# qcraftai/gedepth

Measured on AMD Instinct MI355X. Metric: training img/s (whole node), KITTI-shaped 352x1120 synthetic batches, higher is better.
Workload: dtype bf16; 1 GPU; depthformer_swint_v: DepthFormer-SwinT + GEDepth-Vanilla, 352x1120, 8 img/GPU, full train step; global_batch=8, parallelism=dp1, allreduce_dtype=fp32, layout=nhwc, window_attention=bf16 mfma, params=53516992, hip_graph=off

## Files before the change

gedepth_amd/csrc/conv3x3.hip:

```cpp
#include "common.h"
#include <stdlib.h>

typedef __bf16 cv_bf16x8 __attribute__((ext_vector_type(8)));
typedef float cv_f32x16 __attribute__((ext_vector_type(16)));

#define CV_TH 8
#define CV_TW 32
#define CV_KC 32
#define CV_PITCH 40
#define CV_HALO ((CV_TH + 2) * (CV_TW + 2))
#define CV_NT 64
#define CV_IN_PIECES (CV_HALO * 4)
#define CV_W_PIECES (9 * CV_NT * 4)

__global__ void __launch_bounds__(256, 2) conv3x3_nhwc_k(const bf16_t* __restrict__ x, const bf16_t* __restrict__ w, const float* __restrict__ bias,
                                                         bf16_t* __restrict__ y, int H, int W, int Cin, int Cout, int n_ntiles, float slope,
                                                         int act) {
  __shared__ __attribute__((aligned(16))) bf16_t smem[CV_HALO * CV_PITCH + 9 * CV_NT * CV_PITCH];
  bf16_t* in_tile = smem;
  bf16_t* w_tile = smem + CV_HALO * CV_PITCH;
  const int tid = threadIdx.x, lane = tid & 63, wv = tid >> 6;
  const int tx0 = blockIdx.x * CV_TW, ty0 = blockIdx.y * CV_TH;
  const int n = blockIdx.z / n_ntiles, n0 = (blockIdx.z - n * n_ntiles) * CV_NT;
  const bf16_t* xn = x + (long)n * H * W * Cin;

  int in_src[6], in_dst[6], w_src[9], w_dst[9];
#pragma unroll
  for (int i = 0; i < 6; ++i) {
    const int p = tid + i * 256;
    in_src[i] = -1; in_dst[i] = 0;
    if (p < CV_IN_PIECES) {
      const int pix = p >> 2, part = p & 3;
      const int iy = pix / (CV_TW + 2), ix = pix - iy * (CV_TW + 2);
      const int gy = ty0 + iy - 1, gx = tx0 + ix - 1;
      in_dst[i] = pix * CV_PITCH + part * 8;
      in_src[i] = (gy >= 0 && gy < H && gx >= 0 && gx < W) ? (gy * W + gx) * Cin + part * 8 : -2;
    }
  }
#pragma unroll
  for (int i = 0; i < 9; ++i) {
    const int p = tid + i * 256;
    const int row = p >> 2, part = p & 3;
    const int tap = row / CV_NT, co = row - tap * CV_NT;
    w_dst[i] = row * CV_PITCH + part * 8;
    w_src[i] = (n0 + co < Cout) ? ((n0 + co) * 9 + tap) * Cin + part * 8 : -2;
  }
  uint4 pin[6], pw[9];
  const uint4 zero4 = make_uint4(0, 0, 0, 0);
#define CV_PREFETCH(C0)                                                                          \
  _Pragma("unroll") for (int i = 0; i < 6; ++i) { pin[i] = zero4; if (in_src[i] >= 0) pin[i] = *(const uint4*)(xn + in_src[i] + (C0)); } \
  _Pragma("unroll") for (int i = 0; i < 9; ++i) { pw[i] = zero4; if (w_src[i] >= 0) pw[i] = *(const uint4*)(w + w_src[i] + (C0)); }
#define CV_PARK()                                                                                \
  _Pragma("unroll") for (int i = 0; i < 6; ++i) if (in_src[i] != -1) *(uint4*)(in_tile + in_dst[i]) = pin[i];             \
  _Pragma("unroll") for (int i = 0; i < 9; ++i) *(uint4*)(w_tile + w_dst[i]) = pw[i];

  cv_f32x16 acc[2][2];
#pragma unroll
  for (int a = 0; a < 2; ++a)
#pragma unroll
    for (int b = 0; b < 2; ++b) acc[a][b] = 0.f;
  const int m = lane & 31, kg = lane >> 5;
  const int a_base0 = ((2 * wv) * (CV_TW + 2) + m) * CV_PITCH + kg * 8;
  const int b_base = m * CV_PITCH + kg * 8;

  CV_PREFETCH(0)
  CV_PARK()
  __syncthreads();
  for (int c0 = 0; c0 < Cin; c0 += CV_KC) {
    const bool more = c0 + CV_KC < Cin;
    if (more) { CV_PREFETCH(c0 + CV_KC) }
    {
      cv_bf16x8 A[2][2], B[2][2];
      auto frags = [&](int set, int it) {
        const int tap = it >> 1, ks = it & 1, r = tap / 3, s = tap - 3 * r;
        const int ao = a_base0 + (r * (CV_TW + 2) + s) * CV_PITCH + ks * 16;
        A[set][0] = *(const cv_bf16x8*)(in_tile + ao);
        A[set][1] = *(const cv_bf16x8*)(in_tile + ao + (CV_TW + 2) * CV_PITCH);
        const int bo = b_base + tap * CV_NT * CV_PITCH + ks * 16;
        B[set][0] = *(const cv_bf16x8*)(w_tile + bo);
        B[set][1] = *(const cv_bf16x8*)(w_tile + bo + 32 * CV_PITCH);
      };
      frags(0, 0);
#pragma unroll
      for (int it = 0; it < 18; ++it) {
        if (it < 17) frags((it + 1) & 1, it + 1);
        __builtin_amdgcn_sched_barrier(0);
        const int c = it & 1;
        acc[0][0] = __builtin_amdgcn_mfma_f32_32x32x16_bf16(A[c][0], B[c][0], acc[0][0], 0, 0, 0);
        acc[0][1] = __builtin_amdgcn_mfma_f32_32x32x16_bf16(A[c][0], B[c][1], acc[0][1], 0, 0, 0);
        acc[1][0] = __builtin_amdgcn_mfma_f32_32x32x16_bf16(A[c][1], B[c][0], acc[1][0], 0, 0, 0);
        acc[1][1] = __builtin_amdgcn_mfma_f32_32x32x16_bf16(A[c][1], B[c][1], acc[1][1], 0, 0, 0);
        __builtin_amdgcn_sched_barrier(0);
      }
    }
    __syncthreads();
    if (more) { CV_PARK() }
    __syncthreads();
  }
#undef CV_PREFETCH
#undef CV_PARK

  bf16_t* ot = smem + wv * (64 * 72);
#pragma unroll
  for (int mb = 0; mb < 2; ++mb)
#pragma unroll
    for (int nb = 0; nb < 2; ++nb) {
      const int co = nb * 32 + m;
      const float bv = (bias && n0 + co < Cout) ? bias[n0 + co] : 0.f;
#pragma unroll
      for (int r = 0; r < 16; ++r) {
        float v = acc[mb][nb][r] + bv;
        if (act) v = v > 0.f ? v : v * slope;
        const int px = (r & 3) + 8 * (r >> 2) + 4 * kg;
        ot[(mb * 32 + px) * 72 + co] = __builtin_bit_cast(bf16_t, (__bf16)v);
      }
    }
  __builtin_amdgcn_wave_barrier();
#pragma unroll
  for (int it = 0; it < 8; ++it) {
    const int p = it * 8 + (lane >> 3), piece = lane & 7;
    const int gy = ty0 + 2 * wv + (p >> 5), gx = tx0 + (p & 31);
    if (gy < H && gx < W && n0 + piece * 8 < Cout)
      *(uint4*)(y + (((long)n * H + gy) * W + gx) * Cout + n0 + piece * 8) = *(const uint4*)(ot + p * 72 + piece * 8);
  }
}

#define CD_TH 16
#define CD_TW 32
#define CD_HP ((CD_TH + 2) * (CD_TW + 2))
#define CD_HCH 39
#define CD_WCH 36
#define CD_HB (CD_HCH * 1024)
#define CD_BUF (80 * 1024)
#define CD_NCH (CD_HCH + CD_WCH)
#define CD_SLOTS 10
#define CD_LDS(T, p) ((__attribute__((address_space(3))) T*)(p))
#define CD_GLB(p) ((const __attribute__((address_space(1))) void*)(p))

__device__ __attribute__((aligned(16))) uint32_t cd_zero16[4] = {0, 0, 0, 0};

__global__ void __launch_bounds__(512, 1) conv3x3_nhwc_dma_k(const bf16_t* __restrict__ x, const bf16_t* __restrict__ w, const float* __restrict__ bias,
                                                             bf16_t* __restrict__ y, int H, int W, int Cin, int Cout, int n_ntiles, float slope,
                                                             int act) {
  __shared__ __attribute__((aligned(1024))) unsigned char smem[2 * CD_BUF];
  const int tid = threadIdx.x, lane = tid & 63;
  const int wv = __builtin_amdgcn_readfirstlane(tid >> 6);
  const int tx0 = blockIdx.x * CD_TW, ty0 = blockIdx.y * CD_TH;
  const int n = blockIdx.z / n_ntiles, n0 = (blockIdx.z - n * n_ntiles) * CV_NT;
  const unsigned char* xn = (const unsigned char*)(x + (long)n * H * W * Cin);
  const unsigned char* wb = (const unsigned char*)w;

  unsigned goff[CD_SLOTS];
#pragma unroll
  for (int i = 0; i < CD_SLOTS; ++i) {
    const int ch = wv + 8 * i;
    unsigned off = ~0u;
    if (ch < CD_HCH) {
      const int q = ch * 64 + lane, hp = q >> 2, piece = (q & 3) ^ ((hp >> 2) & 3);
      if (hp < CD_HP) {
        const int iy = hp / (CD_TW + 2), ix = hp - iy * (CD_TW + 2);
        const int gy = ty0 + iy - 1, gx = tx0 + ix - 1;
        if (gy >= 0 && gy < H && gx >= 0 && gx < W) off = (unsigned)(((gy * W + gx) * Cin + piece * 8) * 2);
      }
    } else if (ch < CD_NCH) {
      const int q = (ch - CD_HCH) * 64 + lane, row = q >> 2, piece = (q & 3) ^ ((row >> 2) & 3);
      const int tap = row >> 6, co = row & 63;
      if (n0 + co < Cout) off = (unsigned)((((n0 + co) * 9 + tap) * Cin + piece * 8) * 2);
    }
    goff[i] = off;
  }
  auto dma = [&](int i, int c0, int buf) {
    const int ch = wv + 8 * i;
    const unsigned char* base = ch < CD_HCH ? xn : wb;
    const unsigned char* p = goff[i] == ~0u ? (const unsigned char*)cd_zero16 : base + (size_t)(goff[i] + (unsigned)(c0 * 2));
    const unsigned ldst = (unsigned)(uintptr_t)CD_LDS(unsigned char, smem + buf * CD_BUF + ch * 1024);
    asm volatile("s_mov_b32 m0, %0\n\ts_nop 0\n\tglobal_load_lds_dwordx4 %1, off" :: "s"(ldst), "v"(p) : "memory", "m0");
  };

  cv_f32x16 acc[2][2];
#pragma unroll
  for (int a = 0; a < 2; ++a)
#pragma unroll
    for (int b = 0; b < 2; ++b) acc[a][b] = 0.f;
  const int m = lane & 31, kg = lane >> 5;
  int abase[9][2];
#pragma unroll
  for (int tap = 0; tap < 9; ++tap)
#pragma unroll
    for (int mb = 0; mb < 2; ++mb) {
      const int hp = (2 * wv + mb + tap / 3) * (CD_TW + 2) + m + tap % 3;
      abase[tap][mb] = hp * 64 + ((kg ^ ((hp >> 2) & 3)) << 4);
    }
  const int bbase = CD_HB + m * 64 + ((kg ^ ((m >> 2) & 3)) << 4);

#pragma unroll
  for (int i = 0; i < CD_SLOTS; ++i) dma(i, 0, 0);
  asm volatile("s_waitcnt vmcnt(0)" ::: "memory");
  int buf = 0;
  for (int c0 = 0; c0 < Cin; c0 += CV_KC) {
    asm volatile("" ::: "memory");
    __builtin_amdgcn_s_barrier();
    asm volatile("" ::: "memory");
    const int cn = c0 + CV_KC < Cin ? c0 + CV_KC : c0;
    const unsigned char* base = smem + buf * CD_BUF;
    cv_bf16x8 A[2][2], B[2][2];
    A[0][0] = *(const cv_bf16x8*)(base + abase[0][0]); A[0][1] = *(const cv_bf16x8*)(base + abase[0][1]);
    B[0][0] = *(const cv_bf16x8*)(base + bbase); B[0][1] = *(const cv_bf16x8*)(base + bbase + 2048);
#pragma unroll
    for (int g = 0; g < 18; ++g) {
      const int cs = g & 1, ns = cs ^ 1;
      if (g < 17) {
        const int tap = (g + 1) >> 1, kx = ((g + 1) & 1) << 5;
        A[ns][0] = *(const cv_bf16x8*)(base + (abase[tap][0] ^ kx)); A[ns][1] = *(const cv_bf16x8*)(base + (abase[tap][1] ^ kx));
        B[ns][0] = *(const cv_bf16x8*)(base + (bbase ^ kx) + tap * 4096); B[ns][1] = *(const cv_bf16x8*)(base + (bbase ^ kx) + tap * 4096 + 2048);
      }
      __builtin_amdgcn_sched_barrier(0);
      if (!(g & 1)) dma(g >> 1, cn, buf ^ 1);
      acc[0][0] = __builtin_amdgcn_mfma_f32_32x32x16_bf16(A[cs][0], B[cs][0], acc[0][0], 0, 0, 0);
      acc[0][1] = __builtin_amdgcn_mfma_f32_32x32x16_bf16(A[cs][0], B[cs][1], acc[0][1], 0, 0, 0);
      acc[1][0] = __builtin_amdgcn_mfma_f32_32x32x16_bf16(A[cs][1], B[cs][0], acc[1][0], 0, 0, 0);
      acc[1][1] = __builtin_amdgcn_mfma_f32_32x32x16_bf16(A[cs][1], B[cs][1], acc[1][1], 0, 0, 0);
    }
    dma(9, cn, buf ^ 1);
    asm volatile("s_waitcnt vmcnt(0)" ::: "memory");
    buf ^= 1;
  }
  __builtin_amdgcn_s_barrier();
  asm volatile("" ::: "memory");

  bf16_t* ot = (bf16_t*)smem + wv * (64 * 72);
#pragma unroll
  for (int mb = 0; mb < 2; ++mb)
#pragma unroll
    for (int nb = 0; nb < 2; ++nb) {
      const int co = nb * 32 + m;
      const float bv = (bias && n0 + co < Cout) ? bias[n0 + co] : 0.f;
#pragma unroll
      for (int r = 0; r < 16; ++r) {
        float v = acc[mb][nb][r] + bv;
        if (act) v = v > 0.f ? v : v * slope;
        const int px = (r & 3) + 8 * (r >> 2) + 4 * kg;
        ot[(mb * 32 + px) * 72 + co] = __builtin_bit_cast(bf16_t, (__bf16)v);
      }
    }
  __builtin_amdgcn_wave_barrier();
#pragma unroll
  for (int it = 0; it < 8; ++it) {
    const int p = it * 8 + (lane >> 3), piece = lane & 7;
    const int gy = ty0 + 2 * wv + (p >> 5), gx = tx0 + (p & 31);
    if (gy < H && gx < W && n0 + piece * 8 < Cout)
      *(uint4*)(y + (((long)n * H + gy) * W + gx) * Cout + n0 + piece * 8) = *(const uint4*)(ot + p * 72 + piece * 8);
  }
}

extern "C" int ge_conv3x3_nhwc_fwd(const void* x, const void* w, const float* bias, void* y, int N, int H, int W, int Cin, int Cout, int act,
                                   float slope, int dtype, void* stream) {
  if (!x || !w || !y || N < 0 || H <= 0 || W <= 0 || Cin <= 0 || Cout <= 0) return GE_ERR_BAD_ARG;
  if (dtype != GE_BF16 || Cin % CV_KC || Cout % 8 || (((uintptr_t)x | (uintptr_t)w | (uintptr_t)y) & 15)) return GE_ERR_UNSUPPORTED;
  if ((long)H * W * Cin >= (1L << 31) || (long)Cout * 9 * Cin >= (1L << 31)) return GE_ERR_UNSUPPORTED;
  if (N == 0) return GE_OK;
  const int ntn = (Cout + CV_NT - 1) / CV_NT;
  const char* ev = getenv("GE_CONV3X3");
  const int variant = ev ? atoi(ev) : 0;
  const int hpad16 = (H + CD_TH - 1) / CD_TH * CD_TH, hpad8 = (H + CV_TH - 1) / CV_TH * CV_TH;
  const bool dma = variant == 2 || (variant == 0 && Cin >= 512 && hpad16 * 8 <= hpad8 * 9);
  if (dma) {
    const dim3 grid((W + CD_TW - 1) / CD_TW, (H + CD_TH - 1) / CD_TH, N * ntn);
    if (grid.y > 65535 || grid.z > 65535) return GE_ERR_UNSUPPORTED;
    conv3x3_nhwc_dma_k<<<grid, 512, 0, ge_stream(stream)>>>((const bf16_t*)x, (const bf16_t*)w, bias, (bf16_t*)y, H, W, Cin, Cout, ntn, slope, act);
    GE_LAUNCH_CHECK();
    return GE_OK;
  }
  const dim3 grid((W + CV_TW - 1) / CV_TW, (H + CV_TH - 1) / CV_TH, N * ntn);
  if (grid.y > 65535 || grid.z > 65535) return GE_ERR_UNSUPPORTED;
  conv3x3_nhwc_k<<<grid, 256, 0, ge_stream(stream)>>>((const bf16_t*)x, (const bf16_t*)w, bias, (bf16_t*)y, H, W, Cin, Cout, ntn, slope, act);
  GE_LAUNCH_CHECK();
  return GE_OK;
}
```

gedepth_amd/csrc/conv3x3_wgrad.hip:

```cpp
#include "common.h"

typedef __bf16 wg_bf16x8 __attribute__((ext_vector_type(8)));
typedef __bf16 wg_bf16x4 __attribute__((ext_vector_type(4)));
typedef float wg_f32x16 __attribute__((ext_vector_type(16)));
#define WG_LDS(T, p) ((__attribute__((address_space(3))) T*)(p))

#define WG_TH 8
#define WG_TW 32
#define WG_HALO ((WG_TH + 2) * (WG_TW + 2))
#define WG_PIX (WG_TH * WG_TW)
#define WG_DY_PIECES (WG_PIX * 8)
#define WG_X_PIECES (WG_HALO * 4)

template <int TAP0, int NTAP>
__device__ __forceinline__ void wg_tile_mfma(const bf16_t* dyh, const bf16_t* xt, wg_f32x16* acc) {
  wg_bf16x8 A[2], B[2][NTAP];
#define WG_RD(P) __builtin_shufflevector(__builtin_amdgcn_ds_read_tr16_b64_v4bf16(WG_LDS(wg_bf16x4, (P))), \
                                         __builtin_amdgcn_ds_read_tr16_b64_v4bf16(WG_LDS(wg_bf16x4, (P) + 4 * 32)), 0, 1, 2, 3, 4, 5, 6, 7)
#define WG_FRAGS(SET, KS)                                                                                   \
  {                                                                                                         \
    constexpr int row_ = (KS) >> 1, xh_ = ((KS) & 1) * 16;                                                  \
    A[SET] = WG_RD(dyh + (row_ * 32 + xh_) * 32);                                                           \
    _Pragma("unroll") for (int j = 0; j < NTAP; ++j) {                                                     \
      const int r_ = (TAP0 + j) / 3, s_ = (TAP0 + j) - 3 * r_;                                              \
      B[SET][j] = WG_RD(xt + ((row_ + r_) * (WG_TW + 2) + xh_ + s_) * 32);                                  \
    }                                                                                                       \
  }
#define WG_STEP(KS)                                                                                         \
  {                                                                                                         \
    if ((KS) < 15) WG_FRAGS(((KS) + 1) & 1, ((KS) + 1) & 15)                                                \
    __builtin_amdgcn_sched_barrier(0);                                                                      \
    _Pragma("unroll") for (int j = 0; j < NTAP; ++j)                                                       \
      acc[j] = __builtin_amdgcn_mfma_f32_32x32x16_bf16(A[(KS) & 1], B[(KS) & 1][j], acc[j], 0, 0, 0);       \
    __builtin_amdgcn_sched_barrier(0);                                                                      \
  }
  WG_FRAGS(0, 0)
  WG_STEP(0) WG_STEP(1) WG_STEP(2) WG_STEP(3) WG_STEP(4) WG_STEP(5) WG_STEP(6) WG_STEP(7)
  WG_STEP(8) WG_STEP(9) WG_STEP(10) WG_STEP(11) WG_STEP(12) WG_STEP(13) WG_STEP(14) WG_STEP(15)
#undef WG_STEP
#undef WG_FRAGS
#undef WG_RD
}

__global__ void __launch_bounds__(256, 2) conv3x3_wgrad_k(const bf16_t* __restrict__ x, const bf16_t* __restrict__ dy, float* __restrict__ dw, int N, int H,
                                                          int W, int Cin, int Cout, int tiles_x, int tiles_y, int ksplit) {
  __shared__ __attribute__((aligned(16))) bf16_t dy_t[2 * WG_PIX * 32];
  __shared__ __attribute__((aligned(16))) bf16_t x_t[WG_HALO * 32];
  const int tid = threadIdx.x, lane = tid & 63, wv = tid >> 6;
  const int c0 = blockIdx.x * 32, n0 = blockIdx.y * 64;
  const int mb = wv & 1, tap0 = (wv >> 1) ? 5 : 0, ntap = (wv >> 1) ? 4 : 5;
  wg_f32x16 acc[5];
#pragma unroll
  for (int t = 0; t < 5; ++t) acc[t] = 0.f;
  const int tr_pix = (lane >> 5) * 8 + ((lane & 15) >> 2), tr_col = ((lane >> 4) & 1) * 16 + (lane & 3) * 4;
  const int total_tiles = N * tiles_y * tiles_x;
  uint4 pd[8], px[6];
  const uint4 zero4 = make_uint4(0, 0, 0, 0);
  int dy_yx[8], dy_lds[8], x_yx[6], x_lds[6];
  const int dy_ch = n0 + (tid & 7) * 8, x_ch = c0 + (tid & 3) * 8;
#pragma unroll
  for (int i = 0; i < 8; ++i) {
    const int p = tid + i * 256, pix = p >> 3, part = p & 7;
    dy_yx[i] = ((pix >> 5) << 16) | (pix & 31);
    dy_lds[i] = ((part >> 2) * WG_PIX + pix) * 32 + (part & 3) * 8;
  }
#pragma unroll
  for (int i = 0; i < 6; ++i) {
    const int p = tid + i * 256, pix = p >> 2;
    const int iy = pix / (WG_TW + 2), ix = pix - iy * (WG_TW + 2);
    x_yx[i] = p < WG_X_PIECES ? ((iy << 16) | ix) : -1;
    x_lds[i] = (p >> 2) * 32 + (p & 3) * 8;
  }
  const bool dy_ch_ok = dy_ch < Cout;
#define WG_PREFETCH(T)                                                                                       \
  {                                                                                                          \
    const int t_ = __builtin_amdgcn_readfirstlane(T);                                                        \
    const int per_img = tiles_y * tiles_x;                                                                   \
    const int n_ = t_ / per_img, rem_ = t_ - n_ * per_img;                                                   \
    const int tyi = rem_ / tiles_x;                                                                          \
    const int ty0 = tyi * WG_TH, tx0 = (rem_ - tyi * tiles_x) * WG_TW;                                       \
    const bf16_t* dyn = dy + (long)n_ * H * W * Cout + dy_ch;                                                \
    const bf16_t* xn = x + (long)n_ * H * W * Cin + x_ch;                                                    \
    _Pragma("unroll") for (int i = 0; i < 8; ++i) {                                                         \
      const int gy = ty0 + (dy_yx[i] >> 16), gx = tx0 + (dy_yx[i] & 0xffff);                                 \
      pd[i] = zero4;                                                                                         \
      if (gy < H && gx < W && dy_ch_ok) pd[i] = *(const uint4*)(dyn + (gy * W + gx) * Cout);                 \
    }                                                                                                        \
    _Pragma("unroll") for (int i = 0; i < 6; ++i) {                                                         \
      const int gy = ty0 + (x_yx[i] >> 16) - 1, gx = tx0 + (x_yx[i] & 0xffff) - 1;                           \
      px[i] = zero4;                                                                                         \
      if (x_yx[i] >= 0 && gy >= 0 && gy < H && gx >= 0 && gx < W) px[i] = *(const uint4*)(xn + (gy * W + gx) * Cin); \
    }                                                                                                        \
  }
#define WG_PARK()                                                                                            \
  _Pragma("unroll") for (int i = 0; i < 8; ++i) *(uint4*)(dy_t + dy_lds[i]) = pd[i];                        \
  _Pragma("unroll") for (int i = 0; i < 6; ++i) {                                                           \
    if (x_yx[i] >= 0) *(uint4*)(x_t + x_lds[i]) = px[i];                                                     \
  }
  int t = blockIdx.z;
  if (t < total_tiles) {
    WG_PREFETCH(t)
    WG_PARK()
  }
  __syncthreads();
  for (; t < total_tiles; t += ksplit) {
    const bool more = t + ksplit < total_tiles;
    if (more) { WG_PREFETCH(t + ksplit) }
    const bf16_t* dyh = dy_t + mb * WG_PIX * 32 + tr_pix * 32 + tr_col;
    const bf16_t* xt = x_t + tr_pix * 32 + tr_col;
    if (wv >> 1) wg_tile_mfma<5, 4>(dyh, xt, acc);
    else wg_tile_mfma<0, 5>(dyh, xt, acc);
    __syncthreads();
    if (more) { WG_PARK() }
    __syncthreads();
  }
#undef WG_PREFETCH
#undef WG_PARK
  const int ci = c0 + (lane & 31);
#pragma unroll
  for (int j = 0; j < 5; ++j) {
    if (j < ntap) {
      const int tap = tap0 + j;
#pragma unroll
      for (int r = 0; r < 16; ++r) {
        const int co = n0 + mb * 32 + (r & 3) + 8 * (r >> 2) + 4 * (lane >> 5);
        if (co < Cout) atomicAdd(dw + ((long)co * 9 + tap) * Cin + ci, acc[j][r]);
      }
    }
  }
}

extern "C" int ge_conv3x3_nhwc_wgrad(const void* x, const void* dy, float* dw, int N, int H, int W, int Cin, int Cout, int dtype, void* stream) {
  if (!x || !dy || !dw || N < 0 || H <= 0 || W <= 0 || Cin <= 0 || Cout <= 0) return GE_ERR_BAD_ARG;
  if (dtype != GE_BF16 || Cin % 32 || Cout % 8 || (((uintptr_t)x | (uintptr_t)dy) & 15)) return GE_ERR_UNSUPPORTED;
  if (N == 0) return GE_OK;
  const int tiles_x = (W + WG_TW - 1) / WG_TW, tiles_y = (H + WG_TH - 1) / WG_TH;
  const long total = (long)N * tiles_y * tiles_x;
  if (total >= (1L << 31) || (long)H * W * std::max(Cin, Cout) >= (1L << 31)) return GE_ERR_UNSUPPORTED;
  const int blocks_out = (Cin / 32) * ((Cout + 63) / 64);
  const int cus = ge_cu_count();
  if (!cus) return GE_ERR_BAD_ARG;
  long ksplit = (2L * cus) / blocks_out;
  if (ksplit > total) ksplit = total;
  if (ksplit < 1) ksplit = 1;
  if (ksplit > 65535 || (Cout + 63) / 64 > 65535) return GE_ERR_UNSUPPORTED;
  const dim3 grid(Cin / 32, (Cout + 63) / 64, (unsigned)ksplit);
  conv3x3_wgrad_k<<<grid, 256, 0, ge_stream(stream)>>>((const bf16_t*)x, (const bf16_t*)dy, dw, N, H, W, Cin, Cout, tiles_x, tiles_y, (int)ksplit);
  GE_LAUNCH_CHECK();
  return GE_OK;
}
```

Baseline: 169.7 img/s.

## Add 16x16x32 MFMA variants for 3x3 conv forward and weight-grad kernels

Templates the forward conv kernels (LDS and DMA paths) on an M16 flag that uses 16x16x32 bf16 MFMA tiles with 4x4 accumulators instead of 32x32x16. It also adds a new weight-gradient kernel built on 16x16 MFMA with transposed LDS reads and a revised swizzle. Heuristics pick the 16x16 path for small-Cin, high-workgroup-count forward convs and for large-pixel-count wgrad, with an env override. The intent is better MFMA issue efficiency and lower LDS pressure on the shapes this model uses, at the cost of more register use and more code paths.

Result: no change. 170.1 img/s, median of 6 (+0.2%).

```diff
diff --git a/gedepth_amd/csrc/conv3x3.hip b/gedepth_amd/csrc/conv3x3.hip
--- a/gedepth_amd/csrc/conv3x3.hip
+++ b/gedepth_amd/csrc/conv3x3.hip
@@ -3,6 +3,7 @@
 
 typedef __bf16 cv_bf16x8 __attribute__((ext_vector_type(8)));
 typedef float cv_f32x16 __attribute__((ext_vector_type(16)));
+typedef float cv_f32x4 __attribute__((ext_vector_type(4)));
 
 #define CV_TH 8
 #define CV_TW 32
@@ -13,6 +14,46 @@
 #define CV_IN_PIECES (CV_HALO * 4)
 #define CV_W_PIECES (9 * CV_NT * 4)
 
+template <bool M16> struct CvAcc { cv_f32x16 v[2][2]; };
+template <> struct CvAcc<true> { cv_f32x4 v[4][4]; };
+
+template <bool M16>
+__device__ __forceinline__ void cv_stage_out(const CvAcc<M16>& acc, bf16_t* ot, const float* bias, int n0, int Cout, int act, float slope, int lane) {
+  if constexpr (M16) {
+    const int m = lane & 15, kq = lane >> 4;
+#pragma unroll
+    for (int nb = 0; nb < 4; ++nb) {
+      const int co = nb * 16 + m;
+      const float bv = (bias && n0 + co < Cout) ? bias[n0 + co] : 0.f;
+#pragma unroll
+      for (int mb = 0; mb < 4; ++mb)
+#pragma unroll
+        for (int r = 0; r < 4; ++r) {
+          float v = acc.v[mb][nb][r] + bv;
+          if (act) v = v > 0.f ? v : v * slope;
+          ot[(mb * 16 + 4 * kq + r) * 72 + co] = __builtin_bit_cast(bf16_t, (__bf16)v);
+        }
+    }
+  } else {
+    const int m = lane & 31, kg = lane >> 5;
+#pragma unroll
+    for (int mb = 0; mb < 2; ++mb)
+#pragma unroll
+      for (int nb = 0; nb < 2; ++nb) {
+        const int co = nb * 32 + m;
+        const float bv = (bias && n0 + co < Cout) ? bias[n0 + co] : 0.f;
+#pragma unroll
+        for (int r = 0; r < 16; ++r) {
+          float v = acc.v[mb][nb][r] + bv;
+          if (act) v = v > 0.f ? v : v * slope;
+          const int px = (r & 3) + 8 * (r >> 2) + 4 * kg;
+          ot[(mb * 32 + px) * 72 + co] = __builtin_bit_cast(bf16_t, (__bf16)v);
+        }
+      }
+  }
+}
+
+template <bool M16>
 __global__ void __launch_bounds__(256, 2) conv3x3_nhwc_k(const bf16_t* __restrict__ x, const bf16_t* __restrict__ w, const float* __restrict__ bias,
                                                          bf16_t* __restrict__ y, int H, int W, int Cin, int Cout, int n_ntiles, float slope,
                                                          int act) {
@@ -54,12 +95,19 @@
   _Pragma("unroll") for (int i = 0; i < 6; ++i) if (in_src[i] != -1) *(uint4*)(in_tile + in_dst[i]) = pin[i];             \
   _Pragma("unroll") for (int i = 0; i < 9; ++i) *(uint4*)(w_tile + w_dst[i]) = pw[i];
 
-  cv_f32x16 acc[2][2];
-#pragma unroll
-  for (int a = 0; a < 2; ++a)
-#pragma unroll
-    for (int b = 0; b < 2; ++b) acc[a][b] = 0.f;
-  const int m = lane & 31, kg = lane >> 5;
+  CvAcc<M16> acc;
+  if constexpr (M16) {
+#pragma unroll
+    for (int a = 0; a < 4; ++a)
+#pragma unroll
+      for (int b = 0; b < 4; ++b) acc.v[a][b] = 0.f;
+  } else {
+#pragma unroll
+    for (int a = 0; a < 2; ++a)
+#pragma unroll
+      for (int b = 0; b < 2; ++b) acc.v[a][b] = 0.f;
+  }
+  const int mw = M16 ? 15 : 31, m = lane & mw, kg = M16 ? lane >> 4 : lane >> 5;
   const int a_base0 = ((2 * wv) * (CV_TW + 2) + m) * CV_PITCH + kg * 8;
   const int b_base = m * CV_PITCH + kg * 8;
 
@@ -69,7 +117,30 @@
   for (int c0 = 0; c0 < Cin; c0 += CV_KC) {
     const bool more = c0 + CV_KC < Cin;
     if (more) { CV_PREFETCH(c0 + CV_KC) }
-    {
+    if constexpr (M16) {
+      cv_bf16x8 A[2][4], B[2][4];
+      auto frags = [&](int set, int tap) {
+        const int r = tap / 3, s = tap - 3 * r;
+        const int ao = a_base0 + (r * (CV_TW + 2) + s) * CV_PITCH;
+#pragma unroll
+        for (int mb = 0; mb < 4; ++mb) A[set][mb] = *(const cv_bf16x8*)(in_tile + ao + ((mb >> 1) * (CV_TW + 2) + (mb & 1) * 16) * CV_PITCH);
+        const int bo = b_base + tap * CV_NT * CV_PITCH;
+#pragma unroll
+        for (int nb = 0; nb < 4; ++nb) B[set][nb] = *(const cv_bf16x8*)(w_tile + bo + nb * 16 * CV_PITCH);
+      };
+      frags(0, 0);
+#pragma unroll
+      for (int tap = 0; tap < 9; ++tap) {
+        if (tap < 8) frags((tap + 1) & 1, tap + 1);
+        __builtin_amdgcn_sched_barrier(0);
+        const int c = tap & 1;
+#pragma unroll
+        for (int mb = 0; mb < 4; ++mb)
+#pragma unroll
+          for (int nb = 0; nb < 4; ++nb) acc.v[mb][nb] = __builtin_amdgcn_mfma_f32_16x16x32_bf16(A[c][mb], B[c][nb], acc.v[mb][nb], 0, 0, 0);
+        __builtin_amdgcn_sched_barrier(0);
+      }
+    } else {
       cv_bf16x8 A[2][2], B[2][2];
       auto frags = [&](int set, int it) {
         const int tap = it >> 1, ks = it & 1, r = tap / 3, s = tap - 3 * r;
@@ -86,10 +157,10 @@
         if (it < 17) frags((it + 1) & 1, it + 1);
         __builtin_amdgcn_sched_barrier(0);
         const int c = it & 1;
-        acc[0][0] = __builtin_amdgcn_mfma_f32_32x32x16_bf16(A[c][0], B[c][0], acc[0][0], 0, 0, 0);
-        acc[0][1] = __builtin_amdgcn_mfma_f32_32x32x16_bf16(A[c][0], B[c][1], acc[0][1], 0, 0, 0);
-        acc[1][0] = __builtin_amdgcn_mfma_f32_32x32x16_bf16(A[c][1], B[c][0], acc[1][0], 0, 0, 0);
-        acc[1][1] = __builtin_amdgcn_mfma_f32_32x32x16_bf16(A[c][1], B[c][1], acc[1][1], 0, 0, 0);
+        acc.v[0][0] = __builtin_amdgcn_mfma_f32_32x32x16_bf16(A[c][0], B[c][0], acc.v[0][0], 0, 0, 0);
+        acc.v[0][1] = __builtin_amdgcn_mfma_f32_32x32x16_bf16(A[c][0], B[c][1], acc.v[0][1], 0, 0, 0);
+        acc.v[1][0] = __builtin_amdgcn_mfma_f32_32x32x16_bf16(A[c][1], B[c][0], acc.v[1][0], 0, 0, 0);
+        acc.v[1][1] = __builtin_amdgcn_mfma_f32_32x32x16_bf16(A[c][1], B[c][1], acc.v[1][1], 0, 0, 0);
         __builtin_amdgcn_sched_barrier(0);
       }
     }
@@ -101,20 +172,7 @@
 #undef CV_PARK
 
   bf16_t* ot = smem + wv * (64 * 72);
-#pragma unroll
-  for (int mb = 0; mb < 2; ++mb)
-#pragma unroll
-    for (int nb = 0; nb < 2; ++nb) {
-      const int co = nb * 32 + m;
-      const float bv = (bias && n0 + co < Cout) ? bias[n0 + co] : 0.f;
-#pragma unroll
-      for (int r = 0; r < 16; ++r) {
-        float v = acc[mb][nb][r] + bv;
-        if (act) v = v > 0.f ? v : v * slope;
-        const int px = (r & 3) + 8 * (r >> 2) + 4 * kg;
-        ot[(mb * 32 + px) * 72 + co] = __builtin_bit_cast(bf16_t, (__bf16)v);
-      }
-    }
+  cv_stage_out<M16>(acc, ot, bias, n0, Cout, act, slope, lane);
   __builtin_amdgcn_wave_barrier();
 #pragma unroll
   for (int it = 0; it < 8; ++it) {
@@ -139,6 +197,7 @@
 
 __device__ __attribute__((aligned(16))) uint32_t cd_zero16[4] = {0, 0, 0, 0};
 
+template <bool M16>
 __global__ void __launch_bounds__(512, 1) conv3x3_nhwc_dma_k(const bf16_t* __restrict__ x, const bf16_t* __restrict__ w, const float* __restrict__ bias,
                                                              bf16_t* __restrict__ y, int H, int W, int Cin, int Cout, int n_ntiles, float slope,
                                                              int act) {
@@ -177,18 +236,27 @@
     asm volatile("s_mov_b32 m0, %0\n\ts_nop 0\n\tglobal_load_lds_dwordx4 %1, off" :: "s"(ldst), "v"(p) : "memory", "m0");
   };
 
-  cv_f32x16 acc[2][2];
-#pragma unroll
-  for (int a = 0; a < 2; ++a)
-#pragma unroll
-    for (int b = 0; b < 2; ++b) acc[a][b] = 0.f;
-  const int m = lane & 31, kg = lane >> 5;
-  int abase[9][2];
+  CvAcc<M16> acc;
+  if constexpr (M16) {
+#pragma unroll
+    for (int a = 0; a < 4; ++a)
+#pragma unroll
+      for (int b = 0; b < 4; ++b) acc.v[a][b] = 0.f;
+  } else {
+#pragma unroll
+    for (int a = 0; a < 2; ++a)
+#pragma unroll
+      for (int b = 0; b < 2; ++b) acc.v[a][b] = 0.f;
+  }
+  const int mw = M16 ? 15 : 31, m = lane & mw, kg = M16 ? lane >> 4 : lane >> 5;
+  constexpr int NMB = M16 ? 4 : 2;
+  int abase[9][NMB];
 #pragma unroll
   for (int tap = 0; tap < 9; ++tap)
 #pragma unroll
-    for (int mb = 0; mb < 2; ++mb) {
-      const int hp = (2 * wv + mb + tap / 3) * (CD_TW + 2) + m + tap % 3;
+    for (int mb = 0; mb < NMB; ++mb) {
+      const int hp = M16 ? (2 * wv + (mb >> 1) + tap / 3) * (CD_TW + 2) + (mb & 1) * 16 + m + tap % 3
+                         : (2 * wv + mb + tap / 3) * (CD_TW + 2) + m + tap % 3;
       abase[tap][mb] = hp * 64 + ((kg ^ ((hp >> 2) & 3)) << 4);
     }
   const int bbase = CD_HB + m * 64 + ((kg ^ ((m >> 2) & 3)) << 4);
@@ -203,23 +271,47 @@
     asm volatile("" ::: "memory");
     const int cn = c0 + CV_KC < Cin ? c0 + CV_KC : c0;
     const unsigned char* base = smem + buf * CD_BUF;
-    cv_bf16x8 A[2][2], B[2][2];
-    A[0][0] = *(const cv_bf16x8*)(base + abase[0][0]); A[0][1] = *(const cv_bf16x8*)(base + abase[0][1]);
-    B[0][0] = *(const cv_bf16x8*)(base + bbase); B[0][1] = *(const cv_bf16x8*)(base + bbase + 2048);
-#pragma unroll
-    for (int g = 0; g < 18; ++g) {
-      const int cs = g & 1, ns = cs ^ 1;
-      if (g < 17) {
-        const int tap = (g + 1) >> 1, kx = ((g + 1) & 1) << 5;
-        A[ns][0] = *(const cv_bf16x8*)(base + (abase[tap][0] ^ kx)); A[ns][1] = *(const cv_bf16x8*)(base + (abase[tap][1] ^ kx));
-        B[ns][0] = *(const cv_bf16x8*)(base + (bbase ^ kx) + tap * 4096); B[ns][1] = *(const cv_bf16x8*)(base + (bbase ^ kx) + tap * 4096 + 2048);
-      }
-      __builtin_amdgcn_sched_barrier(0);
-      if (!(g & 1)) dma(g >> 1, cn, buf ^ 1);
-      acc[0][0] = __builtin_amdgcn_mfma_f32_32x32x16_bf16(A[cs][0], B[cs][0], acc[0][0], 0, 0, 0);
-      acc[0][1] = __builtin_amdgcn_mfma_f32_32x32x16_bf16(A[cs][0], B[cs][1], acc[0][1], 0, 0, 0);
-      acc[1][0] = __builtin_amdgcn_mfma_f32_32x32x16_bf16(A[cs][1], B[cs][0], acc[1][0], 0, 0, 0);
-      acc[1][1] = __builtin_amdgcn_mfma_f32_32x32x16_bf16(A[cs][1], B[cs][1], acc[1][1], 0, 0, 0);
+    if constexpr (M16) {
+      cv_bf16x8 A[2][4], B[2][4];
+#pragma unroll
+      for (int mb = 0; mb < 4; ++mb) A[0][mb] = *(const cv_bf16x8*)(base + abase[0][mb]);
+#pragma unroll
+      for (int nb = 0; nb < 4; ++nb) B[0][nb] = *(const cv_bf16x8*)(base + bbase + nb * 1024);
+#pragma unroll
+      for (int g = 0; g < 9; ++g) {
+        const int cs = g & 1, ns = cs ^ 1;
+        if (g < 8) {
+#pragma unroll
+          for (int mb = 0; mb < 4; ++mb) A[ns][mb] = *(const cv_bf16x8*)(base + abase[g + 1][mb]);
+#pragma unroll
+          for (int nb = 0; nb < 4; ++nb) B[ns][nb] = *(const cv_bf16x8*)(base + bbase + (g + 1) * 4096 + nb * 1024);
+        }
+        __builtin_amdgcn_sched_barrier(0);
+        dma(g, cn, buf ^ 1);
+#pragma unroll
+        for (int mb = 0; mb < 4; ++mb)
+#pragma unroll
+          for (int nb = 0; nb < 4; ++nb) acc.v[mb][nb] = __builtin_amdgcn_mfma_f32_16x16x32_bf16(A[cs][mb], B[cs][nb], acc.v[mb][nb], 0, 0, 0);
+      }
+    } else {
+      cv_bf16x8 A[2][2], B[2][2];
+      A[0][0] = *(const cv_bf16x8*)(base + abase[0][0]); A[0][1] = *(const cv_bf16x8*)(base + abase[0][1]);
+      B[0][0] = *(const cv_bf16x8*)(base + bbase); B[0][1] = *(const cv_bf16x8*)(base + bbase + 2048);
+#pragma unroll
+      for (int g = 0; g < 18; ++g) {
+        const int cs = g & 1, ns = cs ^ 1;
+        if (g < 17) {
+          const int tap = (g + 1) >> 1, kx = ((g + 1) & 1) << 5;
+          A[ns][0] = *(const cv_bf16x8*)(base + (abase[tap][0] ^ kx)); A[ns][1] = *(const cv_bf16x8*)(base + (abase[tap][1] ^ kx));
+          B[ns][0] = *(const cv_bf16x8*)(base + (bbase ^ kx) + tap * 4096); B[ns][1] = *(const cv_bf16x8*)(base + (bbase ^ kx) + tap * 4096 + 2048);
+        }
+        __builtin_amdgcn_sched_barrier(0);
+        if (!(g & 1)) dma(g >> 1, cn, buf ^ 1);
+        acc.v[0][0] = __builtin_amdgcn_mfma_f32_32x32x16_bf16(A[cs][0], B[cs][0], acc.v[0][0], 0, 0, 0);
+        acc.v[0][1] = __builtin_amdgcn_mfma_f32_32x32x16_bf16(A[cs][0], B[cs][1], acc.v[0][1], 0, 0, 0);
+        acc.v[1][0] = __builtin_amdgcn_mfma_f32_32x32x16_bf16(A[cs][1], B[cs][0], acc.v[1][0], 0, 0, 0);
+        acc.v[1][1] = __builtin_amdgcn_mfma_f32_32x32x16_bf16(A[cs][1], B[cs][1], acc.v[1][1], 0, 0, 0);
+      }
     }
     dma(9, cn, buf ^ 1);
     asm volatile("s_waitcnt vmcnt(0)" ::: "memory");
@@ -229,20 +321,7 @@
   asm volatile("" ::: "memory");
 
   bf16_t* ot = (bf16_t*)smem + wv * (64 * 72);
-#pragma unroll
-  for (int mb = 0; mb < 2; ++mb)
-#pragma unroll
-    for (int nb = 0; nb < 2; ++nb) {
-      const int co = nb * 32 + m;
-      const float bv = (bias && n0 + co < Cout) ? bias[n0 + co] : 0.f;
-#pragma unroll
-      for (int r = 0; r < 16; ++r) {
-        float v = acc[mb][nb][r] + bv;
-        if (act) v = v > 0.f ? v : v * slope;
-        const int px = (r & 3) + 8 * (r >> 2) + 4 * kg;
-        ot[(mb * 32 + px) * 72 + co] = __builtin_bit_cast(bf16_t, (__bf16)v);
-      }
-    }
+  cv_stage_out<M16>(acc, ot, bias, n0, Cout, act, slope, lane);
   __builtin_amdgcn_wave_barrier();
 #pragma unroll
   for (int it = 0; it < 8; ++it) {
@@ -263,17 +342,23 @@
   const char* ev = getenv("GE_CONV3X3");
   const int variant = ev ? atoi(ev) : 0;
   const int hpad16 = (H + CD_TH - 1) / CD_TH * CD_TH, hpad8 = (H + CV_TH - 1) / CV_TH * CV_TH;
-  const bool dma = variant == 2 || (variant == 0 && Cin >= 512 && hpad16 * 8 <= hpad8 * 9);
+  const bool auto_dma = Cin >= 512 && hpad16 * 8 <= hpad8 * 9;
+  const bool dma = variant == 2 || variant == 4 || ((variant == 0 || variant == 5) && auto_dma);
+  const long wgs = (long)((W + CV_TW - 1) / CV_TW) * ((H + CV_TH - 1) / CV_TH) * N * ntn;
+  const bool m16 = variant == 3 || variant == 4 || (variant == 0 && !auto_dma && Cin <= 192 && wgs >= 2000);
+  const hipStream_t st = ge_stream(stream);
   if (dma) {
     const dim3 grid((W + CD_TW - 1) / CD_TW, (H + CD_TH - 1) / CD_TH, N * ntn);
     if (grid.y > 65535 || grid.z > 65535) return GE_ERR_UNSUPPORTED;
-    conv3x3_nhwc_dma_k<<<grid, 512, 0, ge_stream(stream)>>>((const bf16_t*)x, (const bf16_t*)w, bias, (bf16_t*)y, H, W, Cin, Cout, ntn, slope, act);
+    if (m16) conv3x3_nhwc_dma_k<true><<<grid, 512, 0, st>>>((const bf16_t*)x, (const bf16_t*)w, bias, (bf16_t*)y, H, W, Cin, Cout, ntn, slope, act);
+    else conv3x3_nhwc_dma_k<false><<<grid, 512, 0, st>>>((const bf16_t*)x, (const bf16_t*)w, bias, (bf16_t*)y, H, W, Cin, Cout, ntn, slope, act);
     GE_LAUNCH_CHECK();
     return GE_OK;
   }
   const dim3 grid((W + CV_TW - 1) / CV_TW, (H + CV_TH - 1) / CV_TH, N * ntn);
   if (grid.y > 65535 || grid.z > 65535) return GE_ERR_UNSUPPORTED;
-  conv3x3_nhwc_k<<<grid, 256, 0, ge_stream(stream)>>>((const bf16_t*)x, (const bf16_t*)w, bias, (bf16_t*)y, H, W, Cin, Cout, ntn, slope, act);
+  if (m16) conv3x3_nhwc_k<true><<<grid, 256, 0, st>>>((const bf16_t*)x, (const bf16_t*)w, bias, (bf16_t*)y, H, W, Cin, Cout, ntn, slope, act);
+  else conv3x3_nhwc_k<false><<<grid, 256, 0, st>>>((const bf16_t*)x, (const bf16_t*)w, bias, (bf16_t*)y, H, W, Cin, Cout, ntn, slope, act);
   GE_LAUNCH_CHECK();
   return GE_OK;
 }
diff --git a/gedepth_amd/csrc/conv3x3_wgrad.hip b/gedepth_amd/csrc/conv3x3_wgrad.hip
--- a/gedepth_amd/csrc/conv3x3_wgrad.hip
+++ b/gedepth_amd/csrc/conv3x3_wgrad.hip
@@ -1,8 +1,10 @@
 #include "common.h"
+#include <stdlib.h>
 
 typedef __bf16 wg_bf16x8 __attribute__((ext_vector_type(8)));
 typedef __bf16 wg_bf16x4 __attribute__((ext_vector_type(4)));
 typedef float wg_f32x16 __attribute__((ext_vector_type(16)));
+typedef float wg_f32x4 __attribute__((ext_vector_type(4)));
 #define WG_LDS(T, p) ((__attribute__((address_space(3))) T*)(p))
 
 #define WG_TH 8
@@ -130,6 +132,151 @@
   }
 }
 
+#define W16_HP 40
+#define W16_HROWS ((WG_TH + 2) * W16_HP)
+
+template <int TAP0, int NTAP>
+__device__ __forceinline__ void wg16_tile_mfma(const bf16_t* dyt, const bf16_t* xt, const int (&aoff)[2], const int (&boff)[3][2][2],
+                                               wg_f32x4 (*acc)[2][2]) {
+  wg_bf16x8 A[2][2], B[2][NTAP];
+#define W16_RD(P0, P1) __builtin_shufflevector(__builtin_amdgcn_ds_read_tr16_b64_v4bf16(WG_LDS(wg_bf16x4, (P0))), \
+                                               __builtin_amdgcn_ds_read_tr16_b64_v4bf16(WG_LDS(wg_bf16x4, (P1))), 0, 1, 2, 3, 4, 5, 6, 7)
+#define W16_FRAGS(T)                                                                                          \
+  {                                                                                                           \
+    constexpr int row_ = (T) >> 1, h_ = (T) & 1;                                                              \
+    if (!h_) {                                                                                                \
+      _Pragma("unroll") for (int b = 0; b < 2; ++b)                                                           \
+        A[row_ & 1][b] = W16_RD(dyt + aoff[b] + row_ * 1024, dyt + aoff[b] + row_ * 1024 + 128);              \
+    }                                                                                                         \
+    _Pragma("unroll") for (int j = 0; j < NTAP; ++j) {                                                        \
+      const int r_ = (TAP0 + j) / 3, s_ = (TAP0 + j) - 3 * r_, R_ = row_ + r_, f_ = h_ ^ (R_ & 1);             \
+      B[(T) & 1][j] = W16_RD(xt + R_ * (W16_HP * 32) + boff[s_][0][f_], xt + R_ * (W16_HP * 32) + boff[s_][1][f_]); \
+    }                                                                                                         \
+  }
+#define W16_STEP(T)                                                                                           \
+  {                                                                                                           \
+    if ((T) < 15) W16_FRAGS((T) + 1)                                                                          \
+    __builtin_amdgcn_sched_barrier(0);                                                                        \
+    _Pragma("unroll") for (int j = 0; j < NTAP; ++j)                                                          \
+      _Pragma("unroll") for (int b = 0; b < 2; ++b)                                                           \
+        acc[j][b][(T) & 1] = __builtin_amdgcn_mfma_f32_16x16x32_bf16(A[((T) >> 1) & 1][b], B[(T) & 1][j], acc[j][b][(T) & 1], 0, 0, 0); \
+    __builtin_amdgcn_sched_barrier(0);                                                                        \
+  }
+  W16_FRAGS(0)
+  W16_STEP(0) W16_STEP(1) W16_STEP(2) W16_STEP(3) W16_STEP(4) W16_STEP(5) W16_STEP(6) W16_STEP(7)
+  W16_STEP(8) W16_STEP(9) W16_STEP(10) W16_STEP(11) W16_STEP(12) W16_STEP(13) W16_STEP(14) W16_STEP(15)
+#undef W16_STEP
+#undef W16_FRAGS
+#undef W16_RD
+}
+
+__global__ void __launch_bounds__(256, 2) conv3x3_wgrad16_k(const bf16_t* __restrict__ x, const bf16_t* __restrict__ dy, float* __restrict__ dw, int N,
+                                                            int H, int W, int Cin, int Cout, int tiles_x, int tiles_y, int ksplit) {
+  __shared__ __attribute__((aligned(16))) bf16_t dy_t[2 * WG_PIX * 32];
+  __shared__ __attribute__((aligned(16))) bf16_t x_t[W16_HROWS * 32];
+  const int tid = threadIdx.x, lane = tid & 63, wv = tid >> 6;
+  const int c0 = blockIdx.x * 32, n0 = blockIdx.y * 64;
+  const int mb = wv & 1, tap0 = (wv >> 1) ? 5 : 0, ntap = (wv >> 1) ? 4 : 5;
+  wg_f32x4 acc[5][2][2];
+#pragma unroll
+  for (int t = 0; t < 5; ++t)
+#pragma unroll
+    for (int a = 0; a < 2; ++a)
+#pragma unroll
+      for (int b = 0; b < 2; ++b) acc[t][a][b] = 0.f;
+  const int kq = lane >> 4, l4 = (lane & 15) >> 2, c4 = (lane & 3) * 4;
+  int aoff[2], boff[3][2][2];
+#pragma unroll
+  for (int b = 0; b < 2; ++b) aoff[b] = (mb * WG_PIX + 8 * kq + l4) * 32 + ((b ^ (kq & 1)) * 16) + c4;
+#pragma unroll
+  for (int s = 0; s < 3; ++s)
+#pragma unroll
+    for (int sec = 0; sec < 2; ++sec) {
+      const int v = s + 8 * kq + l4 + 4 * sec;
+      const int o = v * 32 + ((v >> 3) & 1) * 16 + c4;
+      boff[s][sec][0] = o;
+      boff[s][sec][1] = o ^ 16;
+    }
+  const int total_tiles = N * tiles_y * tiles_x;
+  uint4 pd[8], px[6];
+  const uint4 zero4 = make_uint4(0, 0, 0, 0);
+  int dy_yx[8], dy_lds[8], x_yx[6], x_lds[6];
+  const int dy_ch = n0 + (tid & 7) * 8, x_ch = c0 + (tid & 3) * 8;
+#pragma unroll
+  for (int i = 0; i < 8; ++i) {
+    const int p = tid + i * 256, pix = p >> 3, part = p & 7;
+    dy_yx[i] = ((pix >> 5) << 16) | (pix & 31);
+    dy_lds[i] = ((part >> 2) * WG_PIX + pix) * 32 + ((part & 3) ^ (((pix >> 3) & 1) << 1)) * 8;
+  }
+#pragma unroll
+  for (int i = 0; i < 6; ++i) {
+    const int p = tid + i * 256, pix = p >> 2;
+    const int iy = pix / (WG_TW + 2), ix = pix - iy * (WG_TW + 2), q = iy * W16_HP + ix;
+    x_yx[i] = p < WG_X_PIECES ? ((iy << 16) | ix) : -1;
+    x_lds[i] = q * 32 + ((p & 3) ^ (((q >> 3) & 1) << 1)) * 8;
+  }
+  const bool dy_ch_ok = dy_ch < Cout;
+#define WG_PREFETCH(T)                                                                                       \
+  {                                                                                                          \
+    const int t_ = __builtin_amdgcn_readfirstlane(T);                                                        \
+    const int per_img = tiles_y * tiles_x;                                                                   \
+    const int n_ = t_ / per_img, rem_ = t_ - n_ * per_img;                                                   \
+    const int tyi = rem_ / tiles_x;                                                                          \
+    const int ty0 = tyi * WG_TH, tx0 = (rem_ - tyi * tiles_x) * WG_TW;                                       \
+    const bf16_t* dyn = dy + (long)n_ * H * W * Cout + dy_ch;                                                \
+    const bf16_t* xn = x + (long)n_ * H * W * Cin + x_ch;                                                    \
+    _Pragma("unroll") for (int i = 0; i < 8; ++i) {                                                         \
+      const int gy = ty0 + (dy_yx[i] >> 16), gx = tx0 + (dy_yx[i] & 0xffff);                                 \
+      pd[i] = zero4;                                                                                         \
+      if (gy < H && gx < W && dy_ch_ok) pd[i] = *(const uint4*)(dyn + (gy * W + gx) * Cout);                 \
+    }                                                                                                        \
+    _Pragma("unroll") for (int i = 0; i < 6; ++i) {                                                         \
+      const int gy = ty0 + (x_yx[i] >> 16) - 1, gx = tx0 + (x_yx[i] & 0xffff) - 1;                           \
+      px[i] = zero4;                                                                                         \
+      if (x_yx[i] >= 0 && gy >= 0 && gy < H && gx >= 0 && gx < W) px[i] = *(const uint4*)(xn + (gy * W + gx) * Cin); \
+    }                                                                                                        \
+  }
+#define WG_PARK()                                                                                            \
+  _Pragma("unroll") for (int i = 0; i < 8; ++i) *(uint4*)(dy_t + dy_lds[i]) = pd[i];                        \
+  _Pragma("unroll") for (int i = 0; i < 6; ++i) {                                                           \
+    if (x_yx[i] >= 0) *(uint4*)(x_t + x_lds[i]) = px[i];                                                     \
+  }
+  int t = blockIdx.z;
+  if (t < total_tiles) {
+    WG_PREFETCH(t)
+    WG_PARK()
+  }
+  __syncthreads();
+  for (; t < total_tiles; t += ksplit) {
+    const bool more = t + ksplit < total_tiles;
+    if (more) { WG_PREFETCH(t + ksplit) }
+    if (wv >> 1) wg16_tile_mfma<5, 4>(dy_t, x_t, aoff, boff, acc);
+    else wg16_tile_mfma<0, 5>(dy_t, x_t, aoff, boff, acc);
+    __syncthreads();
+    if (more) { WG_PARK() }
+    __syncthreads();
+  }
+#undef WG_PREFETCH
+#undef WG_PARK
+#pragma unroll
+  for (int j = 0; j < 5; ++j) {
+    if (j < ntap) {
+      const int tap = tap0 + j;
+#pragma unroll
+      for (int a = 0; a < 2; ++a)
+#pragma unroll
+        for (int b = 0; b < 2; ++b) {
+          const int ci = c0 + b * 16 + (lane & 15);
+#pragma unroll
+          for (int r = 0; r < 4; ++r) {
+            const int co = n0 + mb * 32 + a * 16 + 4 * kq + r;
+            if (co < Cout) atomicAdd(dw + ((long)co * 9 + tap) * Cin + ci, acc[j][a][b][r]);
+          }
+        }
+    }
+  }
+}
+
 extern "C" int ge_conv3x3_nhwc_wgrad(const void* x, const void* dy, float* dw, int N, int H, int W, int Cin, int Cout, int dtype, void* stream) {
   if (!x || !dy || !dw || N < 0 || H <= 0 || W <= 0 || Cin <= 0 || Cout <= 0) return GE_ERR_BAD_ARG;
   if (dtype != GE_BF16 || Cin % 32 || Cout % 8 || (((uintptr_t)x | (uintptr_t)dy) & 15)) return GE_ERR_UNSUPPORTED;
@@ -145,7 +292,14 @@
   if (ksplit < 1) ksplit = 1;
   if (ksplit > 65535 || (Cout + 63) / 64 > 65535) return GE_ERR_UNSUPPORTED;
   const dim3 grid(Cin / 32, (Cout + 63) / 64, (unsigned)ksplit);
-  conv3x3_wgrad_k<<<grid, 256, 0, ge_stream(stream)>>>((const bf16_t*)x, (const bf16_t*)dy, dw, N, H, W, Cin, Cout, tiles_x, tiles_y, (int)ksplit);
+  const char* ev = getenv("GE_CONV3X3");
+  const int variant = ev ? atoi(ev) : 0;
+  const long px = (long)N * H * W;
+  const bool m16 = variant == 3 || variant == 4 || (variant == 0 && px >= 40000 && (Cin > 64 || px >= 400000));
+  if (!m16)
+    conv3x3_wgrad_k<<<grid, 256, 0, ge_stream(stream)>>>((const bf16_t*)x, (const bf16_t*)dy, dw, N, H, W, Cin, Cout, tiles_x, tiles_y, (int)ksplit);
+  else
+    conv3x3_wgrad16_k<<<grid, 256, 0, ge_stream(stream)>>>((const bf16_t*)x, (const bf16_t*)dy, dw, N, H, W, Cin, Cout, tiles_x, tiles_y, (int)ksplit);
   GE_LAUNCH_CHECK();
   return GE_OK;
 }
```
